# alexj94/future_urban_scene_generation

Measured on AMD Instinct MI355X. Metric: synthesised vehicle crops/sec @256x256, higher is better.
Workload: dtype f32 tensors; conv contraction as 3 fp16 MFMA products of scaled (hi, lo) operand splits, f32 accumulate (error vs fp64 <= 1.3x the exact-f32 MFMA kernel's: observed 0.96-1.27x over 12 operand scales x 5 layers; range-guarded; exact-f32 leg in precision_legs)

## Files before the change

future_urban_scene_generation_amd/csrc/conv_halo_128.hip:

```cpp
#include "conv_kernel_halo.h"
namespace fusg {
hipError_t launch_halo_128(const HaloK& k, dim3 grid, hipStream_t s, int pk, int mode) { return launch_halo<4,1,1,4>(k, grid, s, pk, mode); }
}
#ifdef FUSG_HALO_STAMPS
extern "C" int fusg_debug_halo_stamps(unsigned long long* out) {
    return hipMemcpyFromSymbol(out, HIP_SYMBOL(fusg::g_halo_stamps), sizeof(unsigned long long) * 64 * 4 * 40) == hipSuccess ? 0 : 1;
}
extern "C" int fusg_debug_halo_stamps_clear(void) {
    static unsigned long long z[64 * 4 * 40];
    return hipMemcpyToSymbol(HIP_SYMBOL(fusg::g_halo_stamps), z, sizeof z) == hipSuccess ? 0 : 1;
}
#endif
```

future_urban_scene_generation_amd/csrc/conv_halo_en_128.hip:

```cpp
#include "conv_kernel_halo.h"
namespace fusg {
hipError_t launch_halo_en_128(const HaloK& k, const EntryK& en, dim3 grid, hipStream_t s) { return launch_halo_en<4,1,1,4>(k, en, grid, s); }
}
```

future_urban_scene_generation_amd/csrc/conv_igemm.hip:

```cpp
#include <stdlib.h>
#include <mutex>
#include "conv_kernel_tapunit.h"
#include "conv_kernel_small.h"
#include "conv_kernel_tapunit_f32.h"

namespace fusg {

__global__ __launch_bounds__(256) void conv_splitk_reduce(const ConvK p, int nphase) {
    const int n4 = p.Cout_pad >> 2;
    const long total = (long)nphase * p.M * n4;
    const long idx = (long)blockIdx.x * 256 + threadIdx.x;
    if (idx >= total) return;
    const int c4 = (int)(idx % n4);
    const long pm = idx / n4;
    const int m = (int)(pm % p.M);
    const int phase = (int)(pm / p.M);
    f32x4 s = {0.f, 0.f, 0.f, 0.f};
    const float* base = p.ws + ((long)phase * p.ksplit * p.M + m) * p.Cout_pad + c4 * 4;
    const long slab = (long)p.M * p.Cout_pad;
    int k = 0;
    for (; k + 8 <= p.ksplit; k += 8) {
        f32x4 v[8];
#pragma unroll
        for (int j = 0; j < 8; ++j) v[j] = *(const f32x4*)(base + (long)(k + j) * slab);
// ... 184 lines not shown
            d->tile = bn == 128 ? FUSG_TILE_64x128 : FUSG_TILE_64x64;
    }
    const TileCfg tc = kTiles[d->tile];
    const long tiles = ((Mr + tc.bm - 1) / tc.bm) * (d->cout_pad / tc.bn) * nphase;
    const int nk = d->k_pad / BK;
    if (d->ksplit <= 0) {
        int ks = 1;
        if (tiles < 192 && nk >= 8) {
            ks = (int)((512 + tiles - 1) / tiles);
            if (ks > nk / 4) ks = nk / 4;
            if (ks > 32) ks = 32;
            if (ks < 1) ks = 1;
        }
        d->ksplit = ks;
    }
    if (d->ksplit <= 1) { d->ksplit = 1; return 0; }
    return (int64_t)nphase * d->ksplit * M * d->cout_pad * (int64_t)sizeof(float);
}

static int column_tile(int cout_pad, int cap, long mt = 0, long min_wg = 0) {
    int bn = cout_pad % 128 == 0 ? 128 : (cout_pad % 64 == 0 ? 64 : 32);
    if (bn > cap) bn = cap;
    while (bn > 32 && mt * (cout_pad / bn) < min_wg) bn /= 2;
    if (const int v = env_switches().halo_bn; (v == 32 || v == 64 || v == 128) && cout_pad % v == 0) bn = v;
    return bn;
}

static int tapunit_offsets(int* uoff, const fusg_conv_desc& d, int unit, int RP) {
    const int upp = d.c0k / unit, nunits = d.kh * d.kw * upp;
    for (int j = 0; j < nunits; ++j) {
        const int tap = j / upp, u = j - tap * upp, ky = tap / d.kw, kx = tap - ky * d.kw;
        uoff[j] = ky * RP + kx * d.c0k + u * unit;
    }
    return nunits;
}

template <class Fn> static void for_each_quadrant_tap(int kh, int kw, Fn fn) {
    for (int q = 0; q < 4; ++q)
        for (int ky = 0; ky < kh; ++ky)
            if (((ky - 1) & 1) == (q >> 1))
                for (int kx = 0; kx < kw; ++kx)
                    if (((kx - 1) & 1) == (q & 1)) fn(q, ky, kx);
}

struct ConvRoute {
    int family;
    int vec_epi;
    SmallCfg sc;
    int mode;
    int bn;
    bool ksw;
    bool s2d;
    int sp;
    int HH, HW;
    int RP, unit;
};

static int route_conv(fusg_conv_desc* d, ConvRoute* r) {
    const bool want_bf16 = d->precision == FUSG_PREC_BF16;
    if (want_bf16) d->precision = FUSG_PREC_F16X3;
    const fusg_tensor& x0 = d->src0;
    FUSG_CHECK(is_nhwc(x0), "conv2d: src0 must be NHWC-physical f32 (sc=1, Cs%%4=0, 16B aligned)");
    const bool has1 = d->src1.data != nullptr;
    if (has1) {
        FUSG_CHECK(is_nhwc(d->src1) && same_nhw(x0, d->src1), "conv2d: src1 must be NHWC-physical with src0's n,h,w");
    }
    FUSG_CHECK(d->bias && d->ktab, "conv2d: bias/ktab missing");
    FUSG_CHECK(d->precision >= FUSG_PREC_F32 && d->precision <= FUSG_PREC_EMU_BF16X2, "conv2d: precision %d", d->precision);
    if (d->precision != FUSG_PREC_F16X3) FUSG_CHECK(d->wpack, "conv2d: wpack missing");
    else FUSG_CHECK(aligned16(d->wpack_h) && aligned16(d->wscale) && d->status,
                    "conv2d: F16X3 needs 16B-aligned wpack_h and wscale, and a status word");
    FUSG_CHECK((((uintptr_t)d->wpack) & 15) == 0 && (((uintptr_t)d->ktab) & 7) == 0, "conv2d: wpack/ktab misaligned");
    FUSG_CHECK(d->k_pad > 0 && d->k_pad % BK == 0, "conv2d: k_pad %d not a positive multiple of %d", d->k_pad, BK);
    FUSG_CHECK(d->cout > 0 && d->cout_pad % 32 == 0 && d->cout <= d->cout_pad, "conv2d: bad cout %d / cout_pad %d", d->cout, d->cout_pad);
    FUSG_CHECK(d->c0k >= 0 && d->c0k % 4 == 0 && d->c0k <= x0.sw, "conv2d: bad c0k %d (src0 Cs %ld)", d->c0k, (long)x0.sw);
    FUSG_CHECK(d->stride == 1 || d->stride == 2, "conv2d: stride %d", d->stride);
    FUSG_CHECK(d->upsample == 0 || d->upsample == 1, "conv2d: upsample %d", d->upsample);
    FUSG_CHECK(d->pad_mode == FUSG_PAD_ZERO || d->pad_mode == FUSG_PAD_REFLECT || d->pad_mode == FUSG_PAD_REPLICATE, "conv2d: pad_mode");
    FUSG_CHECK(!d->tile_list || (d->tile_count > 0 && !d->stats_out), "conv2d: tile_list needs tile_count > 0 and no stats_out");
    FUSG_CHECK(d->pre_op >= 0 && d->pre_op <= FUSG_PRE_AFFINE, "conv2d: pre_op");
    FUSG_CHECK(d->act >= 0 && d->act <= FUSG_ACT_LEAKY02, "conv2d: act");
    if (d->pre_op >= FUSG_PRE_AFFINE_RELU) {
        FUSG_CHECK(d->pre_scale && d->pre_shift && ((((uintptr_t)d->pre_scale) | ((uintptr_t)d->pre_shift)) & 15) == 0 &&
                   d->pre_bstride % 4 == 0, "conv2d: affine pre-op needs 16B-aligned scale/shift");
    }
    const int nphase = d->nphase > 0 ? d->nphase : 1;
    FUSG_CHECK(nphase == 1 || nphase == 4, "conv2d: nphase %d", nphase);
    r->sp = 0;
    if (d->tap_sparse != 0) {
        if (!((d->tap_sparse == 1 || d->tap_sparse == 2) && d->kh == 3 && d->kw == 3 && d->pad_h == 1 && d->pad_w == 1 &&
              d->stride == 1 && d->dil == 1 && d->upsample == 0 && d->pad_mode == FUSG_PAD_ZERO && d->store_mode == FUSG_STORE_D2S && nphase == 1 &&
              d->cout > 0 && d->cout % 128 == 0 && d->cout_pad == d->cout)) {
            set_error("conv2d: tap_sparse %d needs a 3x3 zero-pad 1 stride 1 dil 1 D2S launch with nphase 1 and cout %% 128 == 0 "
                      "(kh %d kw %d pad %d,%d stride %d dil %d store %d nphase %d cout %d)", d->tap_sparse, d->kh, d->kw,
                      d->pad_h, d->pad_w, d->stride, d->dil, d->store_mode, nphase, d->cout);
            return FUSG_ERR_UNSUPPORTED;
        }
    }
    FUSG_CHECK(d->qh > 0 && d->qw > 0, "conv2d: empty output grid");
    FUSG_CHECK(d->q_oy >= 0 && d->q_ox >= 0 && (d->store_mode == FUSG_STORE_NORMAL || (d->q_oy | d->q_ox) == 0) &&
               !(d->stats_out && (d->q_oy | d->q_ox)), "conv2d: q-space origin (%d, %d)", d->q_oy, d->q_ox);
    if (nphase == 1 && d->kh > 0 && d->kw > 0) {
        const long Hv = x0.h << d->upsample, Wv = x0.w << d->upsample;
        FUSG_CHECK(d->dil >= 1 && d->pad_h >= 0 && d->pad_w >= 0 &&
                   (d->pad_mode == FUSG_PAD_ZERO ||
                    ((long)(d->q_oy + d->qh - 1) * d->stride + (long)(d->kh - 1) * d->dil - d->pad_h <= Hv - 1 + d->pad_h &&
                     (long)(d->q_ox + d->qw - 1) * d->stride + (long)(d->kw - 1) * d->dil - d->pad_w <= Wv - 1 + d->pad_w &&
                     d->pad_h <= Hv - 1 && d->pad_w <= Wv - 1)),
                   "conv2d: q window [%d+%d, %d+%d] reaches outside the padded input", d->q_oy, d->qh, d->q_ox, d->qw);
    }
    const long Ml = (long)x0.n * d->qh * d->qw;
    FUSG_CHECK(Ml > 0 && Ml < (1L << 31), "conv2d: M out of range");
    FUSG_CHECK(x0.n * x0.h * x0.w * x0.sw < (1L << 40), "conv2d: src too large");
    const fusg_tensor& o = d->dst;
    FUSG_CHECK(o.data && o.dtype == FUSG_F32 && o.n == x0.n, "conv2d: dst missing / batch mismatch");
    long oh, ow, oc;
    if (d->store_mode == FUSG_STORE_D2S) {
        FUSG_CHECK(d->cout % 4 == 0 && nphase == 1, "conv2d: D2S needs cout%%4==0");
        oh = 2L * d->qh; ow = 2L * d->qw; oc = d->cout / 4;
    } else if (d->store_mode == FUSG_STORE_S2D) {
        FUSG_CHECK(d->qh % 2 == 0 && d->qw % 2 == 0 && nphase == 1, "conv2d: S2D needs even output grid");
        oh = d->qh / 2; ow = d->qw / 2; oc = 4L * d->cout;
    } else {
        FUSG_CHECK(d->store_mode == FUSG_STORE_NORMAL && d->out_sy >= 1 && d->out_sx >= 1, "conv2d: store mode / out stride");
        oh = 0; ow = 0;
        for (int ph = 0; ph < nphase; ++ph) {
            FUSG_CHECK(d->out_oy[ph] >= 0 && d->out_ox[ph] >= 0, "conv2d: negative phase offset");
            const long eh = (long)(d->q_oy + d->qh - 1) * d->out_sy + d->out_oy[ph] + 1, ew = (long)(d->q_ox + d->qw - 1) * d->out_sx + d->out_ox[ph] + 1;
            oh = oh > eh ? oh : eh;
            ow = ow > ew ? ow : ew;
        }
        oc = d->cout;
    }
    FUSG_CHECK(oh <= o.h && ow <= o.w && d->dst_c_off >= 0 && d->dst_c_off + oc <= o.c,
               "conv2d: dst [%ld,%ld,%ld,%ld] too small for output %ldx%ldx%ld at channel offset %d",
               (long)o.n, (long)o.c, (long)o.h, (long)o.w, oc, oh, ow, d->dst_c_off);
    const fusg_tensor* rs[2] = {&d->res0, &d->res1};
    for (int i = 0; i < 2; ++i) {
        if (!rs[i]->data) continue;
        FUSG_CHECK(d->store_mode == FUSG_STORE_NORMAL && rs[i]->dtype == FUSG_F32 && rs[i]->n == o.n &&
                   rs[i]->c >= oc && rs[i]->h >= oh && rs[i]->w >= ow, "conv2d: residual %d shape mismatch", i);
// ... 26 lines not shown
    const int ntaps = d->kh * d->kw;
    if (r->sc.ksplit > 0) { r->family = FUSG_CONV_SMALL; return FUSG_OK; }
    if ((d->precision == FUSG_PREC_F16X3 || d->precision == FUSG_PREC_F32) && getenv("FUSG_NO_POINTWISE") == nullptr && nphase == 1 && d->kh == 1 && d->kw == 1 && d->stride == 1 && d->upsample == 0 && !has1 &&
        d->c0k >= 4 && d->c0k <= 8 && d->ksplit <= 1 && d->store_mode == FUSG_STORE_NORMAL && r->vec_epi && !d->stats_out &&
        d->cout % 4 == 0 && d->pre_op <= FUSG_PRE_ELU && (d->q_oy | d->q_ox) == 0 && !d->tile_list && d->wpack && d->pad_h == 0 &&
        d->pad_w == 0 && 256 % (d->cout_pad >> 2) == 0 && !env_switches().no_halo && !env_switches().no_pointwise) {
        r->family = FUSG_CONV_POINTWISE;
        return FUSG_OK;
    }
    const bool f32_frag = d->precision == FUSG_PREC_F32 && aligned16(d->wfrag_f32) && getenv("FUSG_NO_F32_HALO") == nullptr;
    const bool tap_geom = d->wfrag_order == 2 && nphase == 1 && d->upsample == 0 && d->ksplit <= 1 && !has1 && d->c0k >= 4 &&
                          d->c0k <= 24 && d->kh >= 1 && d->kw >= 1 && d->dil == 1 && d->qh % 8 == 0 && d->qw % 16 == 0 &&
                          d->k_pad >= ntaps * d->c0k && (d->q_oy | d->q_ox) == 0 && !d->tile_list && !env_switches().no_halo;
    if (tap_geom && (f32_frag || (d->precision == FUSG_PREC_F16X3 && aligned16(d->wfrag)))) {
        const bool f32 = f32_frag;
        r->HH = 7 * d->stride + d->kh; r->HW = 15 * d->stride + d->kw;
        r->unit = f32 || d->c0k % 8 ? 4 : 8;
        r->RP = f32 ? r->HW * d->c0k : (r->HW * d->c0k + 127) / 128 * 128;
        const int nunits = ntaps * (d->c0k / r->unit), nsteps = (nunits + 16 / r->unit - 1) / (16 / r->unit);
        const size_t lds = f32 ? (size_t)r->HH * r->RP * sizeof(float) : tapunit_lds_bytes(r->HH, r->RP);
        if (nunits <= (f32 ? 320 : 160) && lds <= 80 * 1024 && r->HH * r->HW * (d->c0k / 4) <= 256 * 8) {
            r->mode = f32 ? 2 : (want_bf16 && aligned16(d->wfrag_bf16) && getenv("FUSG_NO_BF16_TAPUNIT") == nullptr ? 1 : 0);
            r->bn = column_tile(d->cout_pad, !f32 && nsteps <= 4 ? 64 : 128);
            r->family = f32 ? FUSG_CONV_TAPUNIT_F32 : r->mode ? FUSG_CONV_TAPUNIT_BF16 : FUSG_CONV_TAPUNIT;
            return FUSG_OK;
        }
    }
    const bool s2d = d->wfrag_order == 1 && d->stride == 2 && x0.h % 2 == 0 && x0.w % 2 == 0 && d->pad_mode != FUSG_PAD_REPLICATE;
    if ((d->precision == FUSG_PREC_F16X3 || f32_frag) && nphase == 1 && d->ksplit <= 1 &&
        ((d->stride == 1 && d->wfrag_order == 0) || (s2d && d->upsample == 0)) &&
        d->kh >= 1 && d->kw >= 1 && d->dil >= 1 && d->c0k % 32 == 0 && d->c0k > 0 &&
        (!has1 || (d->k_pad / ntaps - d->c0k) % 32 == 0) && d->qh % 8 == 0 && d->qw % 16 == 0 &&
        d->k_pad % ntaps == 0 && aligned16(d->wfrag) && !env_switches().no_halo && (d->q_oy | d->q_ox) == 0) {
        if (s2d && !(d->kh == d->kw && (d->kh == 3 || d->kh == 4) && d->pad_h == 1 && d->pad_w == 1 && d->dil == 1 && !has1)) {
            set_error("conv2d: wfrag_order 1 needs stride 2, k3/k4, pad 1, dil 1, one source");
            return FUSG_ERR_INVALID;
        }
        const int tiles_per_img = (d->qh / 8) * (d->qw / 16);
        if (d->tile_list && d->tile_count > tiles_per_img) {
            set_error("conv2d: tile_count %d > %d patches per image", d->tile_count, tiles_per_img);
            return FUSG_ERR_INVALID;
        }
        r->s2d = s2d;
        r->HH = s2d ? 10 : 8 + (d->kh - 1) * d->dil;
        r->HW = s2d ? 18 : 16 + (d->kw - 1) * d->dil;
        if (halo_fits(r->HH, r->HW)) {
            const long mt = route_n((long)x0.n) * (d->tile_list ? d->tile_count : tiles_per_img);
            r->bn = column_tile(d->cout_pad, ntaps == 1 ? 64 : 128, mt, env_switches().halo_minwg);
            r->ksw = !s2d && !d->tile_list && !env_switches().no_ksplit && mt * (d->cout_pad / r->bn) <= 1024 &&
                     ((r->bn == 32 && ntaps >= 4) || (r->bn == 64 && ntaps >= 2));
            const bool bf = want_bf16 && aligned16(d->wfrag_bf16);
            r->mode = f32_frag ? 2 : (bf ? 1 : 0);
            r->sp = r->mode != 1 ? d->tap_sparse : 0;
            r->family = f32_frag ? FUSG_CONV_HALO_F32 : bf ? FUSG_CONV_HALO_BF16 : (s2d ? FUSG_CONV_HALO_S2D : FUSG_CONV_HALO);
            return FUSG_OK;
        }
    }
    if (d->tile_list) {
        set_error("conv2d: tile_list needs a launch that qualifies for the halo kernel");
        return FUSG_ERR_UNSUPPORTED;
    }
    r->family = d->precision == FUSG_PREC_F16X3 ? FUSG_CONV_GENERIC_F16X3 : FUSG_CONV_GENERIC_F32;
    return FUSG_OK;
}

static hipError_t run_small(ConvK& k, const fusg_conv_desc& d, const SmallCfg& sc, hipStream_t s, int pk) {
    k.MT = (int)sc.mt; k.NT = d.cout_pad / 32;
    k.ksplit = sc.ksplit;
    SmallK h;
    memset(&h, 0, sizeof(h));
    h.c = k;
    h.kh = d.kh; h.kw = d.kw; h.pad_h = d.pad_h; h.pad_w = d.pad_w; h.stride = d.stride;
    h.nch0 = d.c0k / 32; h.nch32 = sc.nch32; h.ntaps = sc.ntaps;
    h.wfrag = (const _Float16*)d.wfrag; h.nt32 = d.cout_pad / 32;
    if (d.wfrag_order == 1) {
        int slab = 0;
        for_each_quadrant_tap(d.kh, d.kw, [&](int, int ky, int kx) { h.tapslab |= (unsigned long long)(slab++) << (4 * (ky * d.kw + kx)); });
    } else {
        for (int tp = 0; tp < sc.ntaps; ++tp) h.tapslab |= (unsigned long long)tp << (4 * tp);
    }
    h.nchw = sc.nchw; h.nimg = sc.nimg; h.rpi = sc.rpi; h.rpi_shift = sc.rpi_shift; h.tpi = sc.tpi; h.wide = sc.wide;
    h.pad_mode = d.pad_mode;
    h.RIN = sc.RIN; h.WIN = sc.WIN; h.NPIX = sc.NPIX;
    auto magic = [](int dv) -> unsigned { return dv < 2 ? 0u : (unsigned)(((1UL << 32) + (unsigned long)dv - 1) / (unsigned long)dv); };
    h.m_wo = magic(d.qw); h.m_hw = magic(d.qh * d.qw); h.m_win = magic(sc.WIN); h.m_rw = magic(sc.RIN * sc.WIN);
    h.m_npix = magic(sc.NPIX); h.m_taps = magic(sc.ntaps); h.m_tpi = magic(sc.tpi);
    return launch_small(h, dim3(k.MT * k.NT, 1, sc.ksplit), s, pk);
}

static hipError_t run_pointwise(const ConvK& k, const fusg_conv_desc& d, hipStream_t s) {
    const int n4 = d.cout_pad >> 2, ppb = PW_ITEMS * 256 / n4;
    hipLaunchKernelGGL(conv_pointwise_small, dim3((unsigned)(((long)k.M + ppb - 1) / ppb)), dim3(256),
                       (size_t)(d.cout_pad * 8 + ppb * 8) * sizeof(float), s, k, k.M);
    return hipGetLastError();
}

template <class H> static dim3 tapunit_block(H& h, const ConvK& k, const fusg_conv_desc& d, const ConvRoute& r) {
    memset(&h, 0, sizeof(h));
    h.c = k;
    h.stride = d.stride; h.pad_h = d.pad_h; h.pad_w = d.pad_w;
    h.HH = r.HH; h.HW = r.HW; h.CP = d.c0k; h.PP = d.c0k; h.RP = r.RP;
    h.nunits = tapunit_offsets(h.uoff, d, r.unit, h.RP);
    h.nt32 = d.cout_pad / 32;
    h.tiles_x = d.qw / 16; h.tiles_per_img = (d.qh / 8) * h.tiles_x;
    h.c.MT = (int)d.src0.n * h.tiles_per_img; h.c.NT = d.cout_pad / r.bn;
    h.c.ksplit = 1;
    if (r.mode != 0) { h.c.wscale = nullptr; h.c.status = nullptr; }
    return dim3(h.c.MT * h.c.NT, 1, 1);
}

static hipError_t run_tapunit(const ConvK& k, const fusg_conv_desc& d, const ConvRoute& r, hipStream_t s, int pk) {
    if (r.mode == 2) {
        TapUnitF h;
        const dim3 grid = tapunit_block(h, k, d, r);
        h.wfrag = (const float*)d.wfrag_f32;
        return r.bn == 128 ? launch_tapunit_f32_128(h, grid, s, pk) : r.bn == 64 ? launch_tapunit_f32_64(h, grid, s, pk)
                                                                                 : launch_tapunit_f32_32(h, grid, s, pk);
    }
    TapUnitK h;
    const dim3 grid = tapunit_block(h, k, d, r);
    h.nsteps = (h.nunits + 16 / r.unit - 1) / (16 / r.unit);
    h.wfrag = (const _Float16*)(r.mode == 1 ? d.wfrag_bf16 : d.wfrag);
    return r.bn == 128 ? launch_tapunit_128(h, grid, s, pk, r.unit, r.mode) : r.bn == 64 ? launch_tapunit_64(h, grid, s, pk, r.unit, r.mode)
                                                                                         : launch_tapunit_32(h, grid, s, pk, r.unit, r.mode);
}

static hipError_t run_halo(const ConvK& k, const fusg_conv_desc& d, const ConvRoute& r, hipStream_t s, int pk, const EntryK* en = nullptr) {
    HaloK h;
    memset(&h, 0, sizeof(h));
    h.c = k;
    h.kh = d.kh; h.kw = d.kw; h.dil = d.dil; h.pad_h = d.pad_h; h.pad_w = d.pad_w;
    h.c1k = d.k_pad / (d.kh * d.kw) - d.c0k;
    h.wfrag = (const _Float16*)(r.mode == 1 ? d.wfrag_bf16 : r.mode == 2 ? d.wfrag_f32 : d.wfrag);
    if (r.mode != 0) { h.c.wscale = nullptr; h.c.status = nullptr; }
    h.nt32 = d.cout_pad / 32;
    h.c.NT = d.cout_pad / r.bn;
    h.c.ksplit = 1;
    h.HH = r.HH; h.HW = r.HW;
    if (r.s2d) {
        h.s2d = 1;
        for_each_quadrant_tap(d.kh, d.kw, [&](int q, int ky, int kx) {
            const int n = h.qtaps[q]++;
            h.qtdy[q][n] = ((ky - 1) >> 1) + 1;
            h.qtdx[q][n] = ((kx - 1) >> 1) + 1;
        });
        for (int q = 1; q < 4; ++q) h.qwoff[q] = h.qwoff[q - 1] + h.qtaps[q - 1];
    }
    h.tiles_x = d.qw / 16; h.tiles_per_img = (d.qh / 8) * h.tiles_x;
    h.c.MT = (int)d.src0.n * h.tiles_per_img;
    if (d.tile_list) {
        h.tile_list = d.tile_list; h.tile_count = d.tile_count;
        h.c.MT = (int)d.src0.n * d.tile_count;
    }
    const dim3 grid(h.c.MT * h.c.NT, 1, 1);
    if (en)
        return r.bn == 128 && !r.ksw ? launch_halo_en_128(h, *en, grid, s)
                                     : r.bn == 32 && r.ksw ? launch_halo_en_32k(h, *en, grid, s) : hipErrorInvalidValue;
    if (r.sp)
        return r.bn == 128 ? launch_halo_ts_128(h, grid, s, pk, r.mode, r.sp)
                           : r.bn == 64 ? (r.ksw ? launch_halo_ts_64k(h, grid, s, pk, r.mode, r.sp) : launch_halo_ts_64(h, grid, s, pk, r.mode, r.sp))
                                        : (r.ksw ? launch_halo_ts_32k(h, grid, s, pk, r.mode, r.sp) : launch_halo_ts_32(h, grid, s, pk, r.mode, r.sp));
    return r.bn == 128 ? launch_halo_128(h, grid, s, pk, r.mode)
                       : r.bn == 64 ? (r.ksw ? launch_halo_64k(h, grid, s, pk, r.mode) : launch_halo_64(h, grid, s, pk, r.mode))
                                    : (r.ksw ? launch_halo_32k(h, grid, s, pk, r.mode) : launch_halo_32(h, grid, s, pk, r.mode));
}

typedef hipError_t (*GenericLaunch)(const ConvK&, dim3, hipStream_t, int, bool);
static const GenericLaunch kGeneric[2][6] = {
    {nullptr, launch_tile_128x128, launch_tile_128x64, launch_tile_128x32, launch_tile_64x64, launch_tile_64x128},
    {nullptr, launch_h3_128x128, launch_h3_128x64, launch_h3_128x32, launch_h3_64x64, launch_h3_64x128}};

}

using namespace fusg;

extern "C" int64_t fusg_conv2d_plan(fusg_conv_desc* d) { return plan_impl(d, nullptr); }

extern "C" int fusg_conv2d_route(const fusg_conv_desc* din) {
    fusg_conv_desc d = *din;
    ConvRoute r;
    const int rc = route_conv(&d, &r);
    return rc != FUSG_OK ? rc : r.family;
}

extern "C" int fusg_conv2d_route_order(const fusg_conv_desc* din, int32_t out[4]) {
    FUSG_CHECK(din != nullptr && out != nullptr, "conv2d_route_order: null argument");
    fusg_conv_desc d = *din;
    ConvRoute r;
    if (const int rc = route_conv(&d, &r); rc != FUSG_OK) return rc;
    const bool generic = r.family == FUSG_CONV_GENERIC_F32 || r.family == FUSG_CONV_GENERIC_F16X3;
    const bool halo = r.family == FUSG_CONV_HALO || r.family == FUSG_CONV_HALO_S2D || r.family == FUSG_CONV_HALO_BF16 ||
                      r.family == FUSG_CONV_HALO_F32;
    const bool tapunit = r.family == FUSG_CONV_TAPUNIT || r.family == FUSG_CONV_TAPUNIT_F32 || r.family == FUSG_CONV_TAPUNIT_BF16;
    out[0] = r.family;
    out[1] = generic ? d.tile : (halo || tapunit ? r.bn : 0);
    out[2] = r.family == FUSG_CONV_SMALL ? r.sc.ksplit : (generic ? d.ksplit : 1);
    out[3] = halo && r.ksw ? 1 : 0;
    return FUSG_OK;
}

static int conv2d_run(const fusg_conv_desc* din, const EntryK* en, void* stream) {
    fusg_conv_desc dd = *din;
    fusg_conv_desc* d = &dd;
    ConvRoute r;
    if (const int rc = route_conv(d, &r); rc != FUSG_OK) return rc;
    FUSG_CHECK(!en || (r.family == FUSG_CONV_HALO && r.mode == 0 && r.sp == 0), "conv2d_entry_nin: not a split-fp16 halo launch");
    hipStream_t s = (hipStream_t)stream;
    const fusg_tensor& x0 = d->src0;
    const fusg_tensor& o = d->dst;
    const bool has1 = d->src1.data != nullptr;
    const int nphase = d->nphase > 0 ? d->nphase : 1;
    const long Ml = (long)x0.n * d->qh * d->qw;
    const TileCfg tc = kTiles[d->tile];
    if (d->ksplit > 1) FUSG_CHECK(d->workspace && (((uintptr_t)d->workspace) & 15) == 0, "conv2d: split-K needs a 16B-aligned workspace");
    if (d->ksplit > 1 && d->splitk_counters)
        FUSG_CHECK((long)((Ml + tc.bm - 1) / tc.bm) * (d->cout_pad / tc.bn) * nphase <= d->splitk_counters_len,
                   "conv2d: %d split-K counters for %ld tiles", d->splitk_counters_len, (long)((Ml + tc.bm - 1) / tc.bm) * (d->cout_pad / tc.bn) * nphase);

    ConvK k;
    memset(&k, 0, sizeof(k));
    k.src0 = (const float*)x0.data; k.src1 = has1 ? (const float*)d->src1.data : (const float*)x0.data;
    k.wpack = d->wpack; k.bias = d->bias; k.ktab = (const int2*)d->ktab;
    k.pre_scale = d->pre_scale; k.pre_shift = d->pre_shift; k.pre_bstride = d->pre_bstride;
    k.dst = (float*)o.data; k.dsn = o.sn; k.dsc = o.sc; k.dsh = o.sh; k.dsw = o.sw;
    if (d->res0.data) { k.res0 = (const float*)d->res0.data; k.r0n = d->res0.sn; k.r0c = d->res0.sc; k.r0h = d->res0.sh; k.r0w = d->res0.sw; }
    if (d->res1.data) { k.res1 = (const float*)d->res1.data; k.r1n = d->res1.sn; k.r1c = d->res1.sc; k.r1h = d->res1.sh; k.r1w = d->res1.sw; }
    k.ws = d->workspace;
    k.counters = d->ksplit > 1 ? d->splitk_counters : nullptr;
    k.qy0 = d->q_oy; k.qx0 = d->q_ox;
    k.zeros = zero_line();
    if (!k.zeros) { set_error("conv2d: cannot allocate the zero line"); return FUSG_ERR_LAUNCH; }
    k.touch_w = env_switches().no_touch ? 0 : 1;
    k.wpack_h = (const _Float16*)d->wpack_h;
    if (d->precision == FUSG_PREC_F16X3) { k.wscale = d->wscale; k.status = d->status; }
    k.round_bits = d->precision == FUSG_PREC_EMU_BF16 ? 8 : (d->precision == FUSG_PREC_EMU_BF16X2 ? 16 : 0);
    k.H = (int)x0.h; k.W = (int)x0.w; k.ups = d->upsample; k.Hv = k.H << k.ups; k.Wv = k.W << k.ups;
    k.Cs0 = (int)x0.sw; k.Cs1 = has1 ? (int)d->src1.sw : (int)x0.sw; k.C0 = d->c0k;
    k.K_pad = d->k_pad; k.nk = d->k_pad / BK; k.Cout = d->cout; k.Cout_pad = d->cout_pad;
    k.stride = d->stride; k.pad_mode = d->pad_mode; k.pre_op = d->pre_op; k.act = d->act; k.store_mode = d->store_mode;
    k.B = (int)x0.n; k.Ho = d->qh; k.Wo = d->qw; k.M = (int)Ml;
    k.MT = (k.M + tc.bm - 1) / tc.bm; k.NT = d->cout_pad / tc.bn;
    k.osy = d->out_sy; k.osx = d->out_sx;
    for (int i = 0; i < 4; ++i) { k.ooy[i] = d->out_oy[i]; k.oox[i] = d->out_ox[i]; }
    k.dst_c_off = d->dst_c_off; k.Cd = d->store_mode == FUSG_STORE_D2S ? d->cout / 4 : d->cout;
    k.ksplit = d->ksplit; k.steps_per_split = (k.nk + d->ksplit - 1) / d->ksplit;
    k.vec_epi = r.vec_epi;
    k.stats = d->stats_out;
    if (d->stats_out) k.stats_slots = d->stats_slots > 0 ? d->stats_slots : (int)(((long)d->qh * d->qw) / 32);
    int pk = PK_NONE;
    k.pre_relu = 0;
// ... 88 lines not shown
```

future_urban_scene_generation_amd/csrc/conv_kernel_halo.h:

```cpp
#pragma once
#include "conv_kernel_h3.h"
#ifndef FUSG_HALO_WAVES
#define FUSG_HALO_WAVES 2
#endif

namespace fusg {

typedef __bf16 bf4 __attribute__((ext_vector_type(4)));
typedef __bf16 bf8 __attribute__((ext_vector_type(8)));

#ifdef FUSG_HALO_STAMPS
__device__ unsigned long long g_halo_stamps[64 * 4 * 40];
#define FUSG_HSTAMP(slot) do { if (blockIdx.x < 64 && (slot) < 40 && lane == 0) g_halo_stamps[(blockIdx.x * 4 + wave) * 40 + (slot)] = __builtin_amdgcn_s_memtime(); } while (0)
#else
#define FUSG_HSTAMP(slot) do {} while (0)
#endif

constexpr int HALO_CH = 32;
constexpr int HALO_PP = 32;

struct HaloK {
    ConvK c;
    int kh, kw, dil, pad_h, pad_w;
    int HH, HW;
// ... 24 lines not shown
    if (two) {
        const f32x4 xb = *(const f32x4*)(up + 4);
#pragma unroll
        for (int e = 0; e < 4; ++e)
#pragma unroll
            for (int j = 0; j < 4; ++j) acc[j] = fmaf(xb[e], w[4 + e][j], fmaf(xa[e], w[e][j], acc[j]));
    } else {
#pragma unroll
        for (int e = 0; e < 4; ++e)
#pragma unroll
            for (int j = 0; j < 4; ++j) acc[j] = fmaf(xa[e], w[e][j], acc[j]);
    }
    f32x4 v;
#pragma unroll
    for (int j = 0; j < 4; ++j) v[j] = fmaf(acc[j], 1.f, bias[j]);
    return v;
}

__device__ __forceinline__ void pix_offsets_yx(const ConvK& p, int b, int oy, int ox, PixOff& o) {
    long Y, X, cq = 0;
    if (p.store_mode == FUSG_STORE_D2S) { Y = 2 * oy; X = 2 * ox; }
    else if (p.store_mode == FUSG_STORE_S2D) { Y = oy >> 1; X = ox >> 1; cq = (long)(((oy & 1) << 1) | (ox & 1)) * p.Cout; }
    else { Y = (long)oy * p.osy + p.ooy[0]; X = (long)ox * p.osx + p.oox[0]; }
    o.d = b * p.dsn + Y * p.dsh + X * p.dsw + (cq + p.dst_c_off) * p.dsc;
    o.r0 = b * p.r0n + Y * p.r0h + X * p.r0w;
    o.r1 = b * p.r1n + Y * p.r1h + X * p.r1w;
}

#ifdef FUSG_HALO_OCC
constexpr int halo_waves(int tm, int tn) { return tm * tn == 1 ? 4 : (tm * tn == 2 ? 3 : FUSG_HALO_WAVES); }
#else
constexpr int halo_waves(int, int) { return FUSG_HALO_WAVES; }
#endif

#ifndef FUSG_BF16_OCC
#define FUSG_BF16_OCC 3
#endif
constexpr bool halo_bf16_dense(int tm, int wm, int pk, int ni, int mode, int ks) {
    return FUSG_BF16_OCC > 2 && mode == 1 && ks == 1 && 32 * tm * wm == 128 &&
           !(tm == 4 && ((pk == PK_AFFINE && ni >= 8) || (pk == PK_NONE && ni >= 10)));
}
constexpr int halo_waves_mode(int tm, int tn, int wm, int pk, int ni, int mode, int ks) {
    return halo_bf16_dense(tm, wm, pk, ni, mode, ks) ? FUSG_BF16_OCC : halo_waves(tm, tn);
}
constexpr unsigned tap_sparse_axis(int sp, int parity) { return sp == 1 ? (parity ? 0x6u : 0x3u) : (parity ? 0x6u : 0x2u); }
constexpr unsigned tap_sparse_mask(int sp, int phase) {
    unsigned m = 0;
    for (int ky = 0; ky < 3; ++ky)
        for (int kx = 0; kx < 3; ++kx)
            if (((tap_sparse_axis(sp, phase >> 1) >> ky) & 1u) && ((tap_sparse_axis(sp, phase & 1) >> kx) & 1u)) m |= 1u << (3 * ky + kx);
    return m;
}

template <int TM, int TN, int WM, int WN, int PK, int NI, int MODE, int KS = 1>
__global__ __launch_bounds__(256, halo_waves_mode(TM, TN, WM, PK, NI, MODE, KS)) void conv_halo_h3(const HaloK hk) {
    constexpr int SP = 0, EN = 0;
    const EntryK en = {};
#include "conv_kernel_halo_body.inc"
}
template <int TM, int TN, int WM, int WN, int PK, int NI, int MODE, int KS, int SP>
__global__ __launch_bounds__(256, halo_waves_mode(TM, TN, WM, PK, NI, MODE, KS)) void conv_halo_ts(const HaloK hk) {
    static_assert(SP != 0, "conv_halo_h3 is the dense kernel");
    constexpr int EN = 0;
    const EntryK en = {};
#include "conv_kernel_halo_body.inc"
}
template <int TM, int TN, int WM, int WN, int KS>
__global__ __launch_bounds__(256, FUSG_HALO_WAVES) void conv_halo_en(const HaloK hk, const EntryK en) {
    constexpr int PK = PK_ELU, NI = 6, MODE = 0, SP = 0, EN = 1;
#include "conv_kernel_halo_body.inc"
}

inline int halo_row_pitch(int HW) { return HW * HALO_PP; }
inline size_t halo_lds_bytes(int HH, int HW) { return (size_t)2 * HH * halo_row_pitch(HW) * sizeof(_Float16); }
inline bool halo_fits(int HH, int HW) { return HH * HW * 8 <= 2560 && halo_lds_bytes(HH, HW) <= 96 * 1024; }

template <int TM, int TN, int WM, int WN, int KS, class Pick>
hipError_t launch_halo_fn(const HaloK& k, dim3 grid, hipStream_t s, int pk, int mode, Pick pick,
                          HaloK* prepared = nullptr, size_t* prepared_lds = nullptr) {
    const int HP = k.HH * k.HW;
    size_t lds = halo_lds_bytes(k.HH, k.HW);
    size_t epi = (size_t)4 * TM * 32 * TN * 32 * sizeof(float);
    {
        const int nit = (HP * 8 + 255) / 256 <= 6 ? 6 : ((HP * 8 + 255) / 256 <= 8 ? 8 : 10);
        if (TM >= 4 && halo_bf16_dense(TM, WM, pk, nit, mode, KS)) epi /= 2;
    }
    if (lds < epi) lds = epi;
    const int touch_off = (int)lds;
    lds += TOUCH_LDS_BYTES;
    const int ni = (HP * 8 + 255) / 256;
    if (!halo_fits(k.HH, k.HW)) return hipErrorInvalidValue;
    const void* fn = pick(ni);
    if (!fn) return hipErrorInvalidValue;
    HaloK kk = k;
    kk.RP = halo_row_pitch(k.HW);
    kk.touch_off = touch_off;
    bool fits = true;
    auto magic = [&fits](long nmax, int d) -> unsigned {
        if (d < 1 || nmax * d >= (1L << 32)) fits = false;
        return d < 2 ? 0u : (unsigned)(((1UL << 32) + (unsigned long)d - 1) / (unsigned long)d);
    };
    const long ntiles = (long)grid.x;
    kk.m_hw = magic(256L * 10 + 255, k.HW);
    kk.m_nt = magic(ntiles, k.c.NT);
    kk.m_tpi = magic(ntiles, k.tiles_per_img);
    kk.m_tx = magic((long)k.tiles_per_img, k.tiles_x);
    if (!fits) return hipErrorInvalidValue;
    if (prepared) { *prepared = kk; *prepared_lds = lds; return hipSuccess; }
    return launch_kernel(fn, grid, lds, 96 * 1024 + TOUCH_LDS_BYTES, kk, s);
}

template <int TM, int TN, int WM, int WN, int KS = 1>
hipError_t launch_halo(const HaloK& k, dim3 grid, hipStream_t s, int pk, int mode) {
    return launch_halo_fn<TM, TN, WM, WN, KS>(k, grid, s, pk, mode, [pk, mode](int ni) {
        return pick_pk(pk, [ni, mode](auto pkc) {
            constexpr int PK = decltype(pkc)::value;
            auto by_ni = [ni](auto mdc) {
                constexpr int MD = decltype(mdc)::value;
                return ni <= 6 ? (const void*)conv_halo_h3<TM, TN, WM, WN, PK, 6, MD, KS>
                     : ni <= 8 ? (const void*)conv_halo_h3<TM, TN, WM, WN, PK, 8, MD, KS>
                               : (const void*)conv_halo_h3<TM, TN, WM, WN, PK, 10, MD, KS>;
            };
            return mode == 2 ? by_ni(std::integral_constant<int, 2>{}) : mode == 1 ? by_ni(std::integral_constant<int, 1>{})
                                                                                   : by_ni(std::integral_constant<int, 0>{});
        });
    });
}
template <int TM, int TN, int WM, int WN, int KS = 1>
hipError_t launch_halo_ts(const HaloK& k, dim3 grid, hipStream_t s, int pk, int mode, int sp) {
    if ((mode != 0 && mode != 2) || (sp != 1 && sp != 2) || k.kh != 3 || k.kw != 3 || k.dil != 1 || k.s2d) return hipErrorInvalidValue;
    return launch_halo_fn<TM, TN, WM, WN, KS>(k, grid, s, pk, mode, [pk, mode, sp](int ni) {
        if (ni > 6) return (const void*)nullptr;
        return pick_pk(pk, [mode, sp](auto pkc) {
            constexpr int PK = decltype(pkc)::value;
            auto by_sp = [sp](auto mdc) {
                constexpr int MD = decltype(mdc)::value;
                return sp == 1 ? (const void*)conv_halo_ts<TM, TN, WM, WN, PK, 6, MD, KS, 1>
                               : (const void*)conv_halo_ts<TM, TN, WM, WN, PK, 6, MD, KS, 2>;
            };
            return mode == 2 ? by_sp(std::integral_constant<int, 2>{}) : by_sp(std::integral_constant<int, 0>{});
        });
    });
}

template <int TM, int TN, int WM, int WN, int KS = 1>
hipError_t launch_halo_en(const HaloK& k, const EntryK& en, dim3 grid, hipStream_t s) {
    if (k.kh != 3 || k.kw != 3 || k.dil != 1 || k.pad_h != 1 || k.pad_w != 1 || k.s2d || k.c1k || k.tile_list || k.c.pad_mode != FUSG_PAD_ZERO ||
        k.c.ups || !k.c.vec_epi)
        return hipErrorInvalidValue;
    const size_t need = ((size_t)en_lds_floats(k.HH, halo_row_pitch(k.HW)) + 6 * 32 * 8 + 9 * (size_t)k.c.C0) * sizeof(float);
    if (need > (size_t)4 * TM * 32 * TN * 32 * sizeof(float)) return hipErrorInvalidValue;
    HaloK kk;
    size_t lds = 0;
    const hipError_t e = launch_halo_fn<TM, TN, WM, WN, KS>(k, grid, s, PK_ELU, 0, [&](int ni) {
        return ni == 6 ? (const void*)conv_halo_en<TM, TN, WM, WN, KS> : (const void*)nullptr; }, &kk, &lds);
    if (e != hipSuccess) return e;
    const void* fn = (const void*)conv_halo_en<TM, TN, WM, WN, KS>;
    if (hipError_t e2 = ensure_dyn_lds(fn, 96 * 1024 + TOUCH_LDS_BYTES); e2 != hipSuccess) return e2;
    void* args[] = {(void*)&kk, (void*)&en};
    return hipLaunchKernel(fn, grid, dim3(256), args, lds, s);
}

hipError_t launch_halo_128(const HaloK&, dim3, hipStream_t, int, int);
hipError_t launch_halo_64(const HaloK&, dim3, hipStream_t, int, int);
hipError_t launch_halo_32(const HaloK&, dim3, hipStream_t, int, int);
hipError_t launch_halo_32k(const HaloK&, dim3, hipStream_t, int, int);
hipError_t launch_halo_64k(const HaloK&, dim3, hipStream_t, int, int);
hipError_t launch_halo_ts_128(const HaloK&, dim3, hipStream_t, int, int, int);
hipError_t launch_halo_ts_64(const HaloK&, dim3, hipStream_t, int, int, int);
hipError_t launch_halo_ts_32(const HaloK&, dim3, hipStream_t, int, int, int);
hipError_t launch_halo_ts_32k(const HaloK&, dim3, hipStream_t, int, int, int);
hipError_t launch_halo_ts_64k(const HaloK&, dim3, hipStream_t, int, int, int);
hipError_t launch_halo_en_128(const HaloK&, const EntryK&, dim3, hipStream_t);
hipError_t launch_halo_en_32k(const HaloK&, const EntryK&, dim3, hipStream_t);

}
```

future_urban_scene_generation_amd/csrc/conv_kernel_halo_body.inc:

```
    constexpr bool BF = MODE == 1, F32 = MODE == 2;
    constexpr int CH = HALO_CH, HPITCH = HALO_PP;
    constexpr int CPP = CH / 4;
    constexpr int LOGC = 3;
    const ConvK& p = hk.c;
    constexpr int BM = 32 * TM * WM;
    constexpr int BN = 32 * TN * WN;
    constexpr int PR = BM / 16;
    static_assert(BM == 128 && WM * WN * KS == 4, "8x16 pixel patch, 4 waves");
    static_assert(KS == 1 || (WM == 1 && TN == 1 && TM == 4), "K split: every wave owns the whole patch and one 32-column tile");
    extern __shared__ __attribute__((aligned(16))) _Float16 smem_h[];
    const int HP = hk.HH * hk.HW;
    _Float16* Ah = smem_h;
    _Float16* Al = Ah + hk.HH * hk.RP;
    float* Af = (float*)smem_h;

    const int t = threadIdx.x;
    const int lane = t & 63;
    const int wave = t >> 6;
    FUSG_HSTAMP(0);
    const int wk = wave / (WM * WN);
    const int wm = (wave % (WM * WN)) / WN, wn = wave % WN;
    const int kc = t & (CPP - 1);

    const int tile = xcd_tile();
// ... 271 lines not shown
    int cgn = 0, tapn = 0, qn = 0, cqn = 0, ntn = ntc;
    const _Float16* wnext = wfr + (long)(s2d ? hk.qwoff[0] : 0) * tapstride;
    int qh = 0, cqh = 0;
    auto next_halo_chunk = [&]() { if (s2d && ++cqh == nchq) { cqh = 0; ++qh; } };

    auto advance_w = [&]() __attribute__((always_inline)) {
        wnext += tapstride;
        if (++tapn == ntn) {
            tapn = 0;
            ++cgn;
            if (s2d) {
                if (++cqn == nchq) { cqn = 0; ++qn; }
                ntn = hk.qtaps[qn & 3];
                wnext = wfr + (long)hk.qwoff[qn & 3] * tapstride + (long)cqn * wstep;
            } else {
                wnext = wfr + (long)cgn * wstep;
            }
        }
    };

    if constexpr (KS > 1) {
        auto wptr = [&](int cgx, int tapx) __attribute__((always_inline)) { return wfr + (long)tapx * tapstride + (long)cgx * wstep; };
        halo_issue(hA, 0, 0, 0);
        if constexpr (SP != 0) { if (wk < ntaps && live(wk)) b_load(bfA, wptr(0, wk)); } else
        if (wk < ntaps) b_load(bfA, wptr(0, wk));
        halo_commit(hA);
        __syncthreads();
        bool odd = false;
        for (int cgx = 0; cgx < nch; ++cgx) {
            if (cgx + 1 < nch) halo_issue(hA, cgx + 1, 0, 0);
            int kyx = 0, kxx = wk;
            while (kxx >= hk.kw) { kxx -= hk.kw; ++kyx; }
            for (int tapx = wk; tapx < ntaps; tapx += KS) {
                int ntap = tapx + KS, ncg = cgx;
                if (ntap >= ntaps) { ntap = wk; ++ncg; }
                const _Float16* wn_ptr = wptr(ncg, ntap);
                if constexpr (SP != 0) {
                    if (!odd) { if (ncg < nch && live(ntap)) b_load(bfB, wn_ptr); if (live(tapx)) compute(kyx * hk.dil, kxx * hk.dil, bfA); }
                    else { if (ncg < nch && live(ntap)) b_load(bfA, wn_ptr); if (live(tapx)) compute(kyx * hk.dil, kxx * hk.dil, bfB); }
                } else {
                if (!odd) { if (ncg < nch) b_load(bfB, wn_ptr); compute(kyx * hk.dil, kxx * hk.dil, bfA); }
                else { if (ncg < nch) b_load(bfA, wn_ptr); compute(kyx * hk.dil, kxx * hk.dil, bfB); }
                }
                odd = !odd;
                kxx += KS;
                while (kxx >= hk.kw) { kxx -= hk.kw; ++kyx; }
            }
            if (cgx + 1 < nch) {
                __syncthreads();
                halo_commit(hA);
                __syncthreads();
            }
        }
    } else {
    halo_issue(hA, 0, 0, 0);
    if constexpr (SP != 0) { if (live(0)) b_load(bfA, wnext); } else
    b_load(bfA, wnext);
    halo_commit(hA);
    __syncthreads();
    auto one_step = [&](const BFrag& use, BFrag& fill) __attribute__((always_inline)) {
        if (tap == 0) FUSG_HSTAMP(1 + 3 * cg);
        if (cg == 1) FUSG_HSTAMP(30 + tap);
        if (tap == 0 && cg + 1 < nch) {
            next_halo_chunk();
            halo_issue(hA, cg + 1, qh, cqh);
        }
        if (cg == 1 && tap < 2 && nch <= 6) FUSG_HSTAMP(20 + 4 * tap);
        advance_w();
        if constexpr (SP != 0) { if (cgn < nch && live(tapn)) b_load(fill, wnext); } else
        if (cgn < nch) b_load(fill, wnext);
        if (cg == 1 && tap < 2 && nch <= 6) FUSG_HSTAMP(21 + 4 * tap);
        int dyp = ky * hk.dil, dxp = kx * hk.dil;
        if (s2d) { dyp = hk.qtdy[qc & 3][tap]; dxp = hk.qtdx[qc & 3][tap]; }
        if constexpr (SP != 0) { if (live(tap)) compute(dyp, dxp, use); } else
        compute(dyp, dxp, use);
        if (cg == 1 && tap < 2 && nch <= 6) FUSG_HSTAMP(22 + 4 * tap);
        ++tap;
        if (++kx == hk.kw) { kx = 0; ++ky; }
        if (tap == ntc) {
            FUSG_HSTAMP(2 + 3 * cg);
            tap = 0; ky = 0; kx = 0;
            if (s2d) { if (++cqc == nchq) { cqc = 0; ++qc; } ntc = hk.qtaps[qc & 3]; }
            if (++cg < nch) {
                __syncthreads();
                halo_commit(hA);
                __syncthreads();
            }
            FUSG_HSTAMP(3 * cg);
        }
    };
    for (;;) {
        one_step(bfA, bfB);
        if (cg >= nch) break;
        one_step(bfB, bfA);
        if (cg >= nch) break;
    }

    }

    if constexpr (!BF && !F32) report_range(p, amax);
    if constexpr (KS > 1) {
        constexpr int RW = 128 / KS, TME = RW / 32;
        [[maybe_unused]] ResRegs<TME, 1> rrk;
        if constexpr (EN != 0) en_res(std::integral_constant<int, TME>{}, rrk, RW * wk, nt * BN + wn * 32);
        __syncthreads();
        float* slabs = (float*)smem_h;
// ... 100 lines not shown
```

Measured before the change: 1543.

## Add column-major tap order to halo conv kernel for A-row reuse

```diff
diff --git a/future_urban_scene_generation_amd/csrc/conv_halo_128.hip b/future_urban_scene_generation_amd/csrc/conv_halo_128.hip
--- a/future_urban_scene_generation_amd/csrc/conv_halo_128.hip
+++ b/future_urban_scene_generation_amd/csrc/conv_halo_128.hip
@@ -1,6 +1,8 @@
 #include "conv_kernel_halo.h"
 namespace fusg {
-hipError_t launch_halo_128(const HaloK& k, dim3 grid, hipStream_t s, int pk, int mode) { return launch_halo<4,1,1,4>(k, grid, s, pk, mode); }
+hipError_t launch_halo_128(const HaloK& k, dim3 grid, hipStream_t s, int pk, int mode, bool colmajor) {
+    return launch_halo<4,1,1,4>(k, grid, s, pk, mode, colmajor);
+}
 }
 #ifdef FUSG_HALO_STAMPS
 extern "C" int fusg_debug_halo_stamps(unsigned long long* out) {
diff --git a/future_urban_scene_generation_amd/csrc/conv_halo_en_128.hip b/future_urban_scene_generation_amd/csrc/conv_halo_en_128.hip
--- a/future_urban_scene_generation_amd/csrc/conv_halo_en_128.hip
+++ b/future_urban_scene_generation_amd/csrc/conv_halo_en_128.hip
@@ -1,4 +1,6 @@
 #include "conv_kernel_halo.h"
 namespace fusg {
-hipError_t launch_halo_en_128(const HaloK& k, const EntryK& en, dim3 grid, hipStream_t s) { return launch_halo_en<4,1,1,4>(k, en, grid, s); }
+hipError_t launch_halo_en_128(const HaloK& k, const EntryK& en, dim3 grid, hipStream_t s, bool colmajor) {
+    return launch_halo_en<4,1,1,4>(k, en, grid, s, colmajor);
 }
+}
diff --git a/future_urban_scene_generation_amd/csrc/conv_igemm.hip b/future_urban_scene_generation_amd/csrc/conv_igemm.hip
--- a/future_urban_scene_generation_amd/csrc/conv_igemm.hip
+++ b/future_urban_scene_generation_amd/csrc/conv_igemm.hip
@@ -260,6 +260,7 @@
     bool ksw;
     bool s2d;
     int sp;
+    bool cm;
     int HH, HW;
     int RP, unit;
 };
@@ -295,6 +296,7 @@
     const int nphase = d->nphase > 0 ? d->nphase : 1;
     FUSG_CHECK(nphase == 1 || nphase == 4, "conv2d: nphase %d", nphase);
     r->sp = 0;
+    r->cm = false;
     if (d->tap_sparse != 0) {
         if (!((d->tap_sparse == 1 || d->tap_sparse == 2) && d->kh == 3 && d->kw == 3 && d->pad_h == 1 && d->pad_w == 1 &&
               d->stride == 1 && d->dil == 1 && d->upsample == 0 && d->pad_mode == FUSG_PAD_ZERO && d->store_mode == FUSG_STORE_D2S && nphase == 1 &&
@@ -427,6 +429,8 @@
             const bool bf = want_bf16 && aligned16(d->wfrag_bf16);
             r->mode = f32_frag ? 2 : (bf ? 1 : 0);
             r->sp = r->mode != 1 ? d->tap_sparse : 0;
+            r->cm = r->bn == 128 && !r->ksw && r->mode == 0 && r->sp == 0 && !s2d && d->kh == 3 && d->kw == 3 && d->dil == 1 &&
+                    getenv("FUSG_NO_HALO_COLMAJOR") == nullptr;
             r->family = f32_frag ? FUSG_CONV_HALO_F32 : bf ? FUSG_CONV_HALO_BF16 : (s2d ? FUSG_CONV_HALO_S2D : FUSG_CONV_HALO);
             return FUSG_OK;
         }
@@ -529,13 +533,13 @@
     }
     const dim3 grid(h.c.MT * h.c.NT, 1, 1);
     if (en)
-        return r.bn == 128 && !r.ksw ? launch_halo_en_128(h, *en, grid, s)
+        return r.bn == 128 && !r.ksw ? launch_halo_en_128(h, *en, grid, s, r.cm)
                                      : r.bn == 32 && r.ksw ? launch_halo_en_32k(h, *en, grid, s) : hipErrorInvalidValue;
     if (r.sp)
         return r.bn == 128 ? launch_halo_ts_128(h, grid, s, pk, r.mode, r.sp)
                            : r.bn == 64 ? (r.ksw ? launch_halo_ts_64k(h, grid, s, pk, r.mode, r.sp) : launch_halo_ts_64(h, grid, s, pk, r.mode, r.sp))
                                         : (r.ksw ? launch_halo_ts_32k(h, grid, s, pk, r.mode, r.sp) : launch_halo_ts_32(h, grid, s, pk, r.mode, r.sp));
-    return r.bn == 128 ? launch_halo_128(h, grid, s, pk, r.mode)
+    return r.bn == 128 ? launch_halo_128(h, grid, s, pk, r.mode, r.cm)
                        : r.bn == 64 ? (r.ksw ? launch_halo_64k(h, grid, s, pk, r.mode) : launch_halo_64(h, grid, s, pk, r.mode))
                                     : (r.ksw ? launch_halo_32k(h, grid, s, pk, r.mode) : launch_halo_32(h, grid, s, pk, r.mode));
 }
@@ -570,7 +574,7 @@
     out[0] = r.family;
     out[1] = generic ? d.tile : (halo || tapunit ? r.bn : 0);
     out[2] = r.family == FUSG_CONV_SMALL ? r.sc.ksplit : (generic ? d.ksplit : 1);
-    out[3] = halo && r.ksw ? 1 : 0;
+    out[3] = halo && r.ksw ? 1 : (halo && r.cm ? 2 : 0);
     return FUSG_OK;
 }
 
diff --git a/future_urban_scene_generation_amd/csrc/conv_kernel_halo.h b/future_urban_scene_generation_amd/csrc/conv_kernel_halo.h
--- a/future_urban_scene_generation_amd/csrc/conv_kernel_halo.h
+++ b/future_urban_scene_generation_amd/csrc/conv_kernel_halo.h
@@ -100,7 +100,9 @@
     return m;
 }
 
-template <int TM, int TN, int WM, int WN, int PK, int NI, int MODE, int KS = 1>
+constexpr bool halo_colmajor_tile(int tm, int ks) { return tm == 4 && ks == 1; }
+
+template <int TM, int TN, int WM, int WN, int PK, int NI, int MODE, int KS = 1, int CM = 0>
 __global__ __launch_bounds__(256, halo_waves_mode(TM, TN, WM, PK, NI, MODE, KS)) void conv_halo_h3(const HaloK hk) {
     constexpr int SP = 0, EN = 0;
     const EntryK en = {};
@@ -109,11 +111,11 @@
 template <int TM, int TN, int WM, int WN, int PK, int NI, int MODE, int KS, int SP>
 __global__ __launch_bounds__(256, halo_waves_mode(TM, TN, WM, PK, NI, MODE, KS)) void conv_halo_ts(const HaloK hk) {
     static_assert(SP != 0, "conv_halo_h3 is the dense kernel");
-    constexpr int EN = 0;
+    constexpr int EN = 0, CM = 0;
     const EntryK en = {};
 #include "conv_kernel_halo_body.inc"
 }
-template <int TM, int TN, int WM, int WN, int KS>
+template <int TM, int TN, int WM, int WN, int KS, int CM = 0>
 __global__ __launch_bounds__(256, FUSG_HALO_WAVES) void conv_halo_en(const HaloK hk, const EntryK en) {
     constexpr int PK = PK_ELU, NI = 6, MODE = 0, SP = 0, EN = 1;
 #include "conv_kernel_halo_body.inc"
@@ -158,11 +160,18 @@
     return launch_kernel(fn, grid, lds, 96 * 1024 + TOUCH_LDS_BYTES, kk, s);
 }
 
+inline bool halo_colmajor_ok(const HaloK& k, int mode) { return mode == 0 && k.kh == 3 && k.kw == 3 && k.dil == 1 && !k.s2d; }
+
 template <int TM, int TN, int WM, int WN, int KS = 1>
-hipError_t launch_halo(const HaloK& k, dim3 grid, hipStream_t s, int pk, int mode) {
-    return launch_halo_fn<TM, TN, WM, WN, KS>(k, grid, s, pk, mode, [pk, mode](int ni) {
-        return pick_pk(pk, [ni, mode](auto pkc) {
+hipError_t launch_halo(const HaloK& k, dim3 grid, hipStream_t s, int pk, int mode, bool colmajor = false) {
+    const bool cm = colmajor && halo_colmajor_tile(TM, KS) && halo_colmajor_ok(k, mode);
+    return launch_halo_fn<TM, TN, WM, WN, KS>(k, grid, s, pk, mode, [pk, mode, cm](int ni) {
+        return pick_pk(pk, [ni, mode, cm](auto pkc) {
             constexpr int PK = decltype(pkc)::value;
+            (void)cm;
+            if constexpr (halo_colmajor_tile(TM, KS)) {
+                if (cm) return ni <= 6 ? (const void*)conv_halo_h3<TM, TN, WM, WN, PK, 6, 0, KS, 1> : (const void*)nullptr;
+            }
             auto by_ni = [ni](auto mdc) {
                 constexpr int MD = decltype(mdc)::value;
                 return ni <= 6 ? (const void*)conv_halo_h3<TM, TN, WM, WN, PK, 6, MD, KS>
@@ -192,7 +201,7 @@
 }
 
 template <int TM, int TN, int WM, int WN, int KS = 1>
-hipError_t launch_halo_en(const HaloK& k, const EntryK& en, dim3 grid, hipStream_t s) {
+hipError_t launch_halo_en(const HaloK& k, const EntryK& en, dim3 grid, hipStream_t s, bool colmajor = false) {
     if (k.kh != 3 || k.kw != 3 || k.dil != 1 || k.pad_h != 1 || k.pad_w != 1 || k.s2d || k.c1k || k.tile_list || k.c.pad_mode != FUSG_PAD_ZERO ||
         k.c.ups || !k.c.vec_epi)
         return hipErrorInvalidValue;
@@ -200,16 +209,19 @@
     if (need > (size_t)4 * TM * 32 * TN * 32 * sizeof(float)) return hipErrorInvalidValue;
     HaloK kk;
     size_t lds = 0;
+    const void* fn = (const void*)conv_halo_en<TM, TN, WM, WN, KS>;
+    if constexpr (halo_colmajor_tile(TM, KS)) {
+        if (colmajor) fn = (const void*)conv_halo_en<TM, TN, WM, WN, KS, 1>;
+    }
     const hipError_t e = launch_halo_fn<TM, TN, WM, WN, KS>(k, grid, s, PK_ELU, 0, [&](int ni) {
-        return ni == 6 ? (const void*)conv_halo_en<TM, TN, WM, WN, KS> : (const void*)nullptr; }, &kk, &lds);
+        return ni == 6 ? fn : (const void*)nullptr; }, &kk, &lds);
     if (e != hipSuccess) return e;
-    const void* fn = (const void*)conv_halo_en<TM, TN, WM, WN, KS>;
     if (hipError_t e2 = ensure_dyn_lds(fn, 96 * 1024 + TOUCH_LDS_BYTES); e2 != hipSuccess) return e2;
     void* args[] = {(void*)&kk, (void*)&en};
     return hipLaunchKernel(fn, grid, dim3(256), args, lds, s);
 }
 
-hipError_t launch_halo_128(const HaloK&, dim3, hipStream_t, int, int);
+hipError_t launch_halo_128(const HaloK&, dim3, hipStream_t, int, int, bool colmajor);
 hipError_t launch_halo_64(const HaloK&, dim3, hipStream_t, int, int);
 hipError_t launch_halo_32(const HaloK&, dim3, hipStream_t, int, int);
 hipError_t launch_halo_32k(const HaloK&, dim3, hipStream_t, int, int);
@@ -219,7 +231,7 @@
 hipError_t launch_halo_ts_32(const HaloK&, dim3, hipStream_t, int, int, int);
 hipError_t launch_halo_ts_32k(const HaloK&, dim3, hipStream_t, int, int, int);
 hipError_t launch_halo_ts_64k(const HaloK&, dim3, hipStream_t, int, int, int);
-hipError_t launch_halo_en_128(const HaloK&, const EntryK&, dim3, hipStream_t);
+hipError_t launch_halo_en_128(const HaloK&, const EntryK&, dim3, hipStream_t, bool colmajor);
 hipError_t launch_halo_en_32k(const HaloK&, const EntryK&, dim3, hipStream_t);
 
 }
diff --git a/future_urban_scene_generation_amd/csrc/conv_kernel_halo_body.inc b/future_urban_scene_generation_amd/csrc/conv_kernel_halo_body.inc
--- a/future_urban_scene_generation_amd/csrc/conv_kernel_halo_body.inc
+++ b/future_urban_scene_generation_amd/csrc/conv_kernel_halo_body.inc
@@ -347,6 +347,77 @@
                 __syncthreads();
             }
         }
+    } else if constexpr (CM != 0) {
+    static_assert(TM == 4 && WM == 1 && KS == 1 && SP == 0 && MODE == 0, "column-major taps: the split-fp16 M-whole wide tile");
+    halo_issue(hA, 0, 0, 0);
+    b_load(bfA, wfr);
+    halo_commit(hA);
+    __syncthreads();
+    int cgc = 0, kxc = 0;
+    auto tap_mfma = [&](auto kyc, const h8 (&ah)[8], const h8 (&al)[8], const BFrag& F) __attribute__((always_inline)) {
+        constexpr int KY = decltype(kyc)::value;
+        h8 bs[TN][2];
+#pragma unroll
+        for (int j = 0; j < TN; ++j)
+#pragma unroll
+            for (int ct = 0; ct < 2; ++ct) bs[j][ct] = scale_m11(F.f[j][ct][0]);
+#pragma unroll
+        for (int term = 0; term < 3; ++term)
+#pragma unroll
+            for (int i = 0; i < 8; ++i)
+#pragma unroll
+                for (int j = 0; j < TN; ++j)
+#pragma unroll
+                    for (int ct = 0; ct < 2; ++ct)
+                        acc[i][2 * j + ct] = __builtin_amdgcn_mfma_f32_16x16x32_f16(
+                            term == 2 ? al[(i + KY) & 7] : ah[(i + KY) & 7], term == 0 ? F.f[j][ct][0] : term == 1 ? F.f[j][ct][1] : bs[j][ct],
+                            acc[i][2 * j + ct], 0, 0, 0);
+    };
+    auto one_column = [&](BFrag& F0, BFrag& F1) __attribute__((always_inline)) {
+        if (kxc == 0) {
+            FUSG_HSTAMP(1 + 3 * cgc);
+            if (cgc + 1 < nch) halo_issue(hA, cgc + 1, 0, 0);
+        }
+        const _Float16* wcol = wfr + (long)kxc * tapstride + (long)cgc * wstep;
+        b_load(F1, wcol + 3 * tapstride);
+        const int hx = (lane & 15) + kxc;
+        const int toff = hx * HPITCH + (((lane >> 4) ^ (((hx >> 2) & 1) << 1)) << 3);
+        h8 ah[8], al[8];
+        auto a_row = [&](auto slotc, int r) __attribute__((always_inline)) {
+            ah[decltype(slotc)::value] = *(const h8*)(Ah + r * hk.RP + toff);
+            al[decltype(slotc)::value] = *(const h8*)(Al + r * hk.RP + toff);
+        };
+        a_row(std::integral_constant<int, 0>{}, 0); a_row(std::integral_constant<int, 1>{}, 1);
+        a_row(std::integral_constant<int, 2>{}, 2); a_row(std::integral_constant<int, 3>{}, 3);
+        a_row(std::integral_constant<int, 4>{}, 4); a_row(std::integral_constant<int, 5>{}, 5);
+        a_row(std::integral_constant<int, 6>{}, 6); a_row(std::integral_constant<int, 7>{}, 7);
+        tap_mfma(std::integral_constant<int, 0>{}, ah, al, F0);
+        __builtin_amdgcn_sched_barrier(0);
+        a_row(std::integral_constant<int, 0>{}, 8);
+        b_load(F0, wcol + 6 * tapstride);
+        tap_mfma(std::integral_constant<int, 1>{}, ah, al, F1);
+        __builtin_amdgcn_sched_barrier(0);
+        a_row(std::integral_constant<int, 1>{}, 9);
+        if (kxc < 2) b_load(F1, wcol + tapstride);
+        else if (cgc + 1 < nch) b_load(F1, wfr + (long)(cgc + 1) * wstep);
+        tap_mfma(std::integral_constant<int, 2>{}, ah, al, F0);
+        if (++kxc == 3) {
+            FUSG_HSTAMP(2 + 3 * cgc);
+            kxc = 0;
+            if (++cgc < nch) {
+                __syncthreads();
+                halo_commit(hA);
+                __syncthreads();
+            }
+            FUSG_HSTAMP(3 * cgc);
+        }
+    };
+    for (;;) {
+        one_column(bfA, bfB);
+        if (cgc >= nch) break;
+        one_column(bfB, bfA);
+        if (cgc >= nch) break;
+    }
     } else {
     halo_issue(hA, 0, 0, 0);
     if constexpr (SP != 0) { if (live(0)) b_load(bfA, wnext); } else
```

After: 1586 (median of 6 runs). +2.8%, better.
